# pyannote/pyannote-video

Measured on AMD Instinct MI355X. Metric: frames/sec end-to-end detect->embed->cluster, 1080p@25fps, higher is better.
Workload: dtype f32 (detector scores, embedder) / f64 (tracker, clustering) / u8 frames; an f16 screening pass with a proven error bound decides which windows the detector's exact f32 chain is evaluated for -- results identical to dense f32 scoring (`dense_scoring`)

## Files before the change

include/pvface.h:

```cpp
#ifndef PVFACE_H
#define PVFACE_H
#include <stdint.h>
#include <stddef.h>

#ifdef __cplusplus
extern "C" {
#endif

typedef uint64_t pvf_handle;
typedef struct { int32_t left, top, right, bottom; } pvf_rect_i32;

const char* pvf_last_error(void);
int32_t pvf_version(void);
int32_t pvf_device_count(int32_t* n);
int32_t pvf_ctx_create(int32_t device, pvf_handle* ctx);
int32_t pvf_ctx_create_prio(int32_t device, int32_t priority_class, pvf_handle* ctx);
int32_t pvf_ctx_destroy(pvf_handle ctx);
int32_t pvf_sync(pvf_handle ctx);

int32_t pvf_load_detector(pvf_handle ctx, const char* path);
int32_t pvf_load_shape_predictor(pvf_handle ctx, const char* path);
int32_t pvf_load_embedder(pvf_handle ctx, const char* path);
int32_t pvf_model_tensor(const char* path, int32_t kind, const char* name, void* out, int64_t cap_bytes, int64_t* nbytes);
int32_t pvf_set_tracker_tables(pvf_handle ctx, const double* mask64, const double* mask_scale, const double* tw64,
// ... 241 lines not shown
                        int32_t decimals, char* out, int64_t cap, int64_t* written);

int32_t pvf_round_rows(const float* x, int64_t n, int32_t decimals, double* out);

int32_t pvf_parse_rows(const char* text, int64_t len, double* out, int64_t cap, int64_t* n_rows, int32_t* n_cols);

int32_t pvf_prof_enable(pvf_handle ctx, int32_t on);
int32_t pvf_prof_reset(pvf_handle ctx);
int32_t pvf_prof_get(pvf_handle ctx, const char* family, double* total_ms, int64_t* launches);

int32_t pvf_debug_pyramid_level(pvf_handle ctx, pvf_handle frame, int32_t upsample, int32_t level,
                                uint8_t* out, int32_t* h, int32_t* w);
int32_t pvf_debug_pyramid_batch(pvf_handle ctx, const pvf_handle* frames, int32_t n, int32_t upsample);
int32_t pvf_debug_level_features(pvf_handle ctx, pvf_handle frame, int32_t upsample, int32_t level,
                                 float* out, int32_t* fh, int32_t* fw);
int32_t pvf_debug_level_plan(pvf_handle ctx, pvf_handle frame, int32_t upsample, int32_t level, int32_t* out8);
int32_t pvf_debug_fhog(pvf_handle ctx, const uint8_t* img, int32_t h, int32_t w, int32_t cell, int32_t pad_r,
                       int32_t pad_c, float* out, int32_t* fh, int32_t* fw);
int32_t pvf_debug_detect_raw(pvf_handle ctx, pvf_handle frame, int32_t upsample, double adjust, float* scores,
                             int32_t* meta , int32_t cap, int32_t* n);
int32_t pvf_debug_detect_raw_many(pvf_handle ctx, const pvf_handle* frames, int32_t n_frames, int32_t batch, int32_t upsample,
                                  double adjust, int32_t* counts, int32_t* rows, int64_t cap, int64_t* total);
int32_t pvf_debug_extract_chip(pvf_handle ctx, pvf_handle frame, const double rect[4], double cs, double sn,
                               int32_t rows, int32_t cols, uint8_t* out);
int32_t pvf_debug_tracker_state(pvf_handle ctx, pvf_handle trk, double* F, double* A, double* B);
int32_t pvf_debug_tracker_scale_state(pvf_handle ctx, pvf_handle trk, double* As, double* Bs);
int32_t pvf_debug_embed_stage(pvf_handle ctx, const uint8_t* chips, int32_t n, int32_t split, int32_t stage, float* out, int32_t dims[3],
                              int32_t* flags);
int32_t pvf_debug_conv(pvf_handle ctx, const int32_t geom[18], const float* in, const float* w, const float* bias, const float* gamma,
                       const float* beta, const float* skip, int32_t split, int32_t force_generic, float* out, int32_t* flags);
// ... 15 lines not shown
```

pyannote-video_amd/csrc/api.hip:

```cpp
#include "pvf_internal.h"
#include <algorithm>
#include <cmath>
#include <cstdlib>
#include <string>
#include <thread>

#define API_BEGIN try {
#define API_END                                                        \
    return 0;                                                          \
    }                                                                  \
    catch (const std::exception& e) { pvf_set_error(e.what()); return -1; } \
    catch (...) { pvf_set_error("unknown error"); return -2; }

#define ENTER(c, h)                                                \
    Ctx* c = pvf_ctx(h);                                           \
    std::lock_guard<std::recursive_mutex> _api_lock(c->api_mu);    \
    HIP_CHECK(hipSetDevice(c->device))
#define ENTER_DET(c, h)                                            \
    Ctx* c = pvf_ctx(h);                                           \
    std::lock_guard<std::recursive_mutex> _det_lock(c->det_mu);    \
    HIP_CHECK(hipSetDevice(c->device))
#define ENTER_BOTH(c, h)                                           \
    Ctx* c = pvf_ctx(h);                                           \
    std::lock_guard<std::recursive_mutex> _det_lock(c->det_mu);    \
// ... 185 lines not shown
    std::vector<Frame> fr;
    for (int i = 0; i < n; ++i) fr.push_back(c->frame(frames[i]));
    det_pyramid_batch(c, fr, upsample);
    API_END
}

extern "C" int32_t pvf_debug_level_features(pvf_handle h, pvf_handle frame, int32_t upsample, int32_t level, float* out, int32_t* fh, int32_t* fw)
{
    API_BEGIN
    ENTER_DET(c, h);
    std::vector<float> buf;
    int a = 0, b = 0;
    det_level_features(c, c->frame(frame), upsample, level, out ? &buf : nullptr, &a, &b);
    *fh = a; *fw = b;
    if (out) memcpy(out, buf.data(), buf.size() * sizeof(float));
    API_END
}

extern "C" int32_t pvf_debug_level_plan(pvf_handle h, pvf_handle frame, int32_t upsample, int32_t level, int32_t* out8)
{
    API_BEGIN
    ENTER_DET(c, h);
    PVF_REQUIRE(out8 != nullptr, "pvf_debug_level_plan: out8 is NULL");
    det_level_plan(c, c->frame(frame), upsample, level, out8);
    API_END
}

extern "C" int32_t pvf_debug_fhog(pvf_handle h, const uint8_t* img, int32_t ih, int32_t iw, int32_t cell, int32_t pad_r, int32_t pad_c,
                                  float* out, int32_t* fh, int32_t* fw)
{
// ... 1020 lines not shown
```

pyannote-video_amd/csrc/detect.hip:

```cpp
#include "detect_ml.h"
#include <algorithm>
#include <thread>
#include <cmath>
#include <cstdlib>

#define RESIZE_MAXS 22
struct RowTab { int32_t top, bottom; double tb, tb1, pad; };
struct ColTab { int32_t left, pad; double lr, lr1, pad2; };

template <int RS, int NSTRIP>
__global__ void __launch_bounds__(256) resize_rows_k(const uint8_t* const* __restrict__ in_ptrs, const uint8_t* __restrict__ in_base,
                                                     size_t in_stride, int in_rb, int ih, int iw, uint8_t* __restrict__ out,
                                                     size_t out_stride, int out_rb, int oh, int ow,
                                                     const RowTab* __restrict__ rows, const ColTab* __restrict__ cols)
{
    constexpr int MAXS = (RS == 16) ? RESIZE_MAXS : (RS * 5) / 4 + 3;
    __shared__ uint32_t s_rows[4][MAXS][64];
    __shared__ uint32_t s_out[4][64];
    const int lane = threadIdx.x & 63;
    const int wave = __builtin_amdgcn_readfirstlane(threadIdx.x >> 6);
    const int c0 = blockIdx.x * 256 + wave * 64;
    const int b = blockIdx.z;
    if (c0 >= ow) return;
    const int c = min(c0 + lane, ow - 1);
// ... 1007 lines not shown
                    memcpy(out->data() + ((size_t)y * d.fw + x) * PVF_FHOG_STRIDE + 4 * j, dev.data() + feat_at(y, j, x, d.fwp), 4 * sizeof(float));
    }
    HIP_CHECK(hipStreamSynchronize(c->det_stream));
}

void det_level_plan(Ctx* c, const Frame& f, int upsample, int level, int32_t out[8])
{
    PVF_REQUIRE(c->det.loaded, "detector not loaded");
    MlPlan* p = ml_plan(c, f.h, f.w, upsample, 1);
    PVF_REQUIRE(level >= 0 && level < (int)p->lv.size(), "pyramid level out of range");
    const LvDesc& d = p->lv[level];
    const int32_t v[8] = {d.h, d.w, d.hog_nr, d.hog_nc, d.chunk_rows, d.chunks, d.roll_rows, d.roll_nseg};
    memcpy(out, v, sizeof v);
}

static bool raw_less(const RawDet& x, const RawDet& y)
{
    if (x.score != y.score) return x.score > y.score;
    if (x.filter != y.filter) return x.filter < y.filter;
    if (x.level != y.level) return x.level < y.level;
    if (x.r != y.r) return x.r < y.r;
    return x.c < y.c;
}

static void decode_candidates(const DetectorModel& m, int upsample, const CandRec* q, int n, std::vector<RawDet>& v);

static void screen_verdict(Ctx* c, const int* ctl)
{
    if (!c->det_screen || c->det_screen_suspended) return;
    c->screen_listed += std::min(ctl[SCR_FLAGGED], c->screen_list_cap);
    if (ctl[SCR_FLAGGED] > c->screen_list_cap || ctl[SCR_VIOLATION] != 0) {
        HIP_CHECK(hipStreamSynchronize(c->det_stream));
        throw ScreenRetry();
    }
}

struct CandLayout { ScratchLayout lay; ScratchSlot<int> counts; ScratchSlot<CandRec> cands; };
static CandLayout cand_layout(int frames, int per_frame)
{
    CandLayout l;
    l.counts = l.lay.take<int>(frames + SCR_CTL_INTS, 64);
    l.cands = l.lay.take<CandRec>((size_t)frames * per_frame, 64);
    l.lay.pad(64);
    return l;
}

void det_run_batch(Ctx* c, const std::vector<Frame>& frames, int upsample, double adjust, std::vector<std::vector<RawDet>>& raw_sorted)
{
    const DetectorModel& m = c->det;
    PVF_REQUIRE(m.loaded, "detector not loaded");
    PVF_REQUIRE(!frames.empty(), "no frames");
    const int B = (int)frames.size();
    const int cap = c->det_cand_cap;
    const CandLayout cl = cand_layout(B, cap);
    c->s_cand.ensure(cl.lay.bytes());
    int* d_counts = cl.counts.in(c->s_cand); CandRec* d_cands = cl.cands.in(c->s_cand);
    HIP_CHECK(hipMemsetAsync(d_counts, 0, (size_t)(B + SCR_CTL_INTS) * sizeof(int), c->det_stream));
    ScoreParams sp;
    for (int f = 0; f < 8; ++f) sp.thresh[f] = f < m.n_filters ? (float)((double)m.thresh[f] + adjust) : 3.0e38f;
// ... 142 lines not shown
```

pyannote-video_amd/csrc/detect_ml.h:

```cpp
#pragma once
#include "pvf_internal.h"
#include "fhog_dev.h"

#define ML_MAX 32
struct LvDesc {
    int h, w, rb;
    int cells_nr, cells_nc, visible_nr, visible_nc;
    int fh, fw, hog_nr, hog_nc;
    int fwp;
    int feat_bx, score_bx;
    int valid_score;
    int roll_nseg, roll_rows;
    int strips, chunks, chunk_rows, fused_tasks;
    long long img_off, img_stride;
    long long feat_off, feat_stride;
};
struct MlStarts { int nl; int b0[ML_MAX + 1]; };

#define FEAT_PAD_COLS 52
__host__ __device__ __forceinline__ size_t feat_at(int row, int j, int col, int fwp) { return (((size_t)row * 8 + j) * fwp + col) * 4; }

struct ScoreParams { float thresh[8]; int n_filters; int level; int cap; };
struct CandRec { float score; int32_t filter, level, r, c; };

// ... 4 lines not shown
static_assert((SCR_GROUP_COLS - 1) + SCR_TAIL_CELLS - (SCR_FILTER_COLS - 1) <= FEAT_PAD_COLS,
              "FEAT_PAD_COLS: the screening pass's tail read leaves a feature row's zero columns");
struct ScreenItem { int32_t lv, b, c_base, r_base, out_rows, ng; };
enum { SCR_CURSOR = 0, SCR_FLAGGED = 1, SCR_VIOLATION = 2, SCR_CTL_INTS = 4 };

struct ScreenPlan {
    ScreenItem* d_items = nullptr;
    int n_items = 0;
    bool usable = false;
    ~ScreenPlan() { if (d_items) (void)hipFree(d_items); }
    ScreenPlan() = default;
    ScreenPlan(const ScreenPlan&) = delete;
    ScreenPlan& operator=(const ScreenPlan&) = delete;
};
void screen_plan_build(ScreenPlan& sp, const std::vector<LvDesc>& lv, int B);
void screen_launch(Ctx* c, const ScreenPlan& sp, const LvDesc* d_lv, int B, const float* feat, const ScoreParams& thr, int* d_counts,
                   CandRec* d_cands, int* ctl);
void screen_prepare_model(DetectorModel& d, const float* w);
```

pyannote-video_amd/csrc/pvf_internal.h:

```cpp
#pragma once
#include <hip/hip_runtime.h>
#include <cstdint>
#include <cstdio>
#include <cstring>
#include <deque>
#include <map>
#include <atomic>
#include <memory>
#include <mutex>
#include <stdexcept>
#include <string>
#include <unordered_map>
#include <vector>
#include "../../include/pvface.h"
#include "scratch_layout.h"
#include "chip_plan.h"
#include "group_blocks.h"

#define PVF_FHOG_STRIDE 32

struct CandOverflow : PvfError { int needed; explicit CandOverflow(int n) : PvfError("detector: candidate buffer overflow"), needed(n) {} };
struct ScreenRetry : PvfError { ScreenRetry() : PvfError("detector: screening pass gave up") {} };

#define HIP_CHECK(expr)                                                                              \
// ... 300 lines not shown
void det_run_many(Ctx* c, const std::vector<Frame>& frames, int batch, int upsample, double adjust,
                  std::vector<std::vector<RawDet>>& raw_sorted, bool nms = false);
void ml_plans_free(Ctx* c);
void ingest_free_all(Ctx* c);
struct ResizeTab { std::vector<int32_t> idx; std::vector<int16_t> coef; };
ResizeTab linear_table(int in, int out);
void render_free_all(Ctx* c);
void tube_free_all(Ctx* c);
void board_free_all(Ctx* c);
void board_thumbs_device(Ctx* c, const pvf_handle* frames, int n, int tw, int th, uint8_t* d_out);
int board_thumbs_per_round(size_t picture_bytes);
void det_nms(const DetectorModel& m, const std::vector<RawDet>& sorted, std::vector<RawDet>& out);
void det_pyramid_level(Ctx* c, const Frame& f, int upsample, int level, std::vector<uint8_t>* out, int* h, int* w);
void det_level_features(Ctx* c, const Frame& f, int upsample, int level, std::vector<float>* out, int* fh, int* fw);
void det_level_plan(Ctx* c, const Frame& f, int upsample, int level, int32_t out[8]);
void det_pyramid_batch(Ctx* c, const std::vector<Frame>& frames, int upsample);
void fhog_debug(Ctx* c, const uint8_t* himg, int h, int w, int cell, int pad_r, int pad_c, std::vector<float>& out, int* fh, int* fw);
void fhog_device(Ctx* c, const uint8_t* d_img, int n, int h, int w, int cell, int pad_r, int pad_c, float* d_feat,
                 DevBuf& hist, DevBuf& norm, size_t img_stride_in = 0);
void fhog1_compact(Ctx* c, const uint8_t* d_chips, int n, uint8_t* d_rec);
void fhog_scale_chips(Ctx* c, const uint8_t* d_chips, int n, float* d_feat);
void fhog_dims(int ih, int iw, int cell, int pad_r, int pad_c, int* fh, int* fw);
ChipJob chip_plan(const Frame& f, const ChipDetails& d);
void chip_extract_batch(Ctx* c, const std::vector<ChipJob>& jobs, uint8_t* d_out );
void transform_batch(Ctx* c, const std::vector<ChipJob>& jobs, uint8_t* d_out);
void transform_launch(Ctx* c, const DevXfJob* d_jobs, int n, int rows, int cols, uint8_t* d_out);
void jitter_check_count(const char* who, int J);
void jitter_plan_rows(int J, uint64_t seed, double* out );
int jitter_faces_per_round(int J);
uint8_t* jitter_scratch(Ctx* c, int faces, int J);
// ... 64 lines not shown
```

pyannote-video_amd/csrc/screen.hip:

```cpp
#include "detect_ml.h"
#include <algorithm>
#include <cmath>
#include <cstring>

typedef _Float16 f16x8 __attribute__((ext_vector_type(8)));
typedef _Float16 f16x2 __attribute__((ext_vector_type(2)));

struct ScreenParams { float flag_at[8]; float lim_lo, lim_hi; int n_items, list_cap; };

#define SCR_B_BYTES (10 * 12 * 64 * 16)
#define SCR_M_STRIDE (12 * 64 * 16)

__device__ __forceinline__ uint32_t pk_f16(float a, float b)
{
    return __builtin_bit_cast(uint32_t, __builtin_amdgcn_cvt_pkrtz(a, b));
}

template <int NG>
__device__ __forceinline__ void screen_walk(const ScreenItem t, const LvDesc* __restrict__ lv, const float* __restrict__ feat_base,
                                            const uint8_t* s_b, const float th_lane, int* __restrict__ ctl, uint2* __restrict__ list,
                                            const int list_cap, u32x4& mx)
{
    constexpr int RSRC_FLAGS = 0x00020000;
    constexpr int FR = 10, FC = 10;
    static_assert(FC == SCR_FILTER_COLS, "detect_ml.h: SCR_FILTER_COLS is this kernel's filter width");
    const int lane = threadIdx.x & 63, i = lane & 15, kq = lane >> 4;
    const int fw = lv[t.lv].fw;
    const long long feat_off = lv[t.lv].feat_off, feat_stride = lv[t.lv].feat_stride;
    const int fwp = lv[t.lv].fwp;
    const float* fb = feat_base + feat_off + (size_t)t.b * feat_stride + feat_at(t.r_base, 0, t.c_base, fwp);
    const int row_bytes = (8 * fwp - t.c_base) * 16;
    const int fh_in = t.out_rows + FR - 1;
    const int c1 = fw - (FC - FC / 2 - 1);
    const int voff = i * 48 + kq * 2 * fwp * 16;
    const int voff2 = voff + fwp * 16;
    const int voff_t = i < 3 ? voff : 0x40000000, voff2_t = i < 3 ? voff2 : 0x40000000;
    f32x4 acc[10][NG];
#pragma unroll
    for (int q = 0; q < 10; ++q)
#pragma unroll
        for (int g = 0; g < NG; ++g) acc[q][g] = (f32x4){0.f, 0.f, 0.f, 0.f};
    const uint8_t* b_lo = s_b + lane * 16;
    const uint8_t* b_hi = s_b + lane * 16 + 5 * SCR_M_STRIDE;
    auto load_cls = [&](int row, int cls, u32x4 (&raw)[NG + 1][2]) {
        const __amdgpu_buffer_rsrc_t rs = __builtin_amdgcn_make_buffer_rsrc((void*)(fb + (size_t)row * 8 * fwp * 4), 0,
                                                                            row < fh_in ? row_bytes : 0, RSRC_FLAGS);
#pragma unroll
        for (int g = 0; g <= NG; ++g) {
            raw[g][0] = __builtin_amdgcn_raw_buffer_load_b128(rs, (g < NG ? voff : voff_t) + cls * 16 + g * 768, 0, 0);
            raw[g][1] = __builtin_amdgcn_raw_buffer_load_b128(rs, (g < NG ? voff2 : voff2_t) + cls * 16 + g * 768, 0, 0);
        }
    };
    auto cvt_frag = [&](const u32x4 (&r)[2]) -> u32x4 {
        u32x4 o;
        o.x = pk_f16(__uint_as_float(r[0].x), __uint_as_float(r[0].y)); o.y = pk_f16(__uint_as_float(r[0].z), __uint_as_float(r[0].w));
        o.z = pk_f16(__uint_as_float(r[1].x), __uint_as_float(r[1].y)); o.w = pk_f16(__uint_as_float(r[1].z), __uint_as_float(r[1].w));
#pragma unroll
        for (int k = 0; k < 4; ++k) mx[k] = __builtin_bit_cast(uint32_t, __builtin_elementwise_max(__builtin_bit_cast(f16x2, mx[k]), __builtin_bit_cast(f16x2, o[k])));
        return o;
    };
    auto shift_bases = [&](u32x4 (&a)[NG + 1]) {
#pragma unroll
        for (int g = 0; g <= NG; ++g) {
#pragma unroll
            for (int e = 0; e < 4; ++e) {
                int fill = 0;
                if (g < NG) fill = __builtin_amdgcn_update_dpp(0, (int)a[g + 1][e], 0x11F , 0xf, 0xf, true);
                a[g][e] = (uint32_t)__builtin_amdgcn_update_dpp(fill, (int)a[g][e], 0x101 , 0xf, 0xf, false);
            }
        }
    };
    auto emit = [&](const f32x4 (&a)[NG], int r_out) {
        float vm = a[0][0];
#pragma unroll
        for (int g = 0; g < NG; ++g)
#pragma unroll
            for (int e = 0; e < 4; ++e) vm = fmaxf(vm, a[g][e]);
        const bool hit = vm >= th_lane;
        if (r_out >= 0 && __builtin_amdgcn_ballot_w64(hit) != 0) {
            const int jc = lane & 15;
            const int sft = jc / 5, f = jc % 5;
            const int r = t.r_base + r_out + FR / 2;
#pragma unroll
            for (int g = 0; g < NG; ++g)
#pragma unroll
                for (int e = 0; e < 4; ++e) {
                    const int cc = t.c_base + 48 * g + 3 * (4 * kq + e) + sft + FC / 2;
                    if (a[g][e] >= th_lane && cc < c1) {
                        const int idx = atomicAdd(&ctl[SCR_FLAGGED], 1);
                        if (idx < list_cap) list[idx] = make_uint2((uint32_t)t.b, ((uint32_t)t.lv << 27) | ((uint32_t)f << 24) | ((uint32_t)r << 12) | (uint32_t)cc);
                    }
                }
        }
    };

    u32x4 A[3][NG + 1];
    {
        u32x4 raw[NG + 1][2];
#pragma unroll
        for (int cls = 0; cls < 3; ++cls) {
            load_cls(0, cls, raw);
#pragma unroll
            for (int g = 0; g <= NG; ++g) A[cls][g] = cvt_frag(raw[g]);
        }
    }
    auto b_frag = [&](int q, int j) -> u32x4 {
        return *reinterpret_cast<const u32x4*>((q < 5 ? b_lo + q * SCR_M_STRIDE : b_hi + (q - 5) * SCR_M_STRIDE) + j * 1024);
    };
    u32x4 bn[10];
#pragma unroll
    for (int q = 0; q < 10; ++q) bn[q] = b_frag(q, 0);
    for (int s = 0; s < fh_in; ++s) {
        u32x4 An[3][NG + 1];
        u32x4 raw[NG + 1][2];
        f32x4 done[NG];
#pragma unroll
        for (int j = 0; j < 12; ++j) {
            const int cls = j % 3;
            if (j > 0 && cls == 0) {
#pragma unroll
                for (int k = 0; k < 3; ++k) shift_bases(A[k]);
            }
            if (j % 4 == 0) load_cls(s + 1, j / 4, raw);
            u32x4 bc[10];
#pragma unroll
            for (int q = 0; q < 10; ++q) bc[q] = bn[q];
#pragma unroll
            for (int q = 0; q < 10; ++q) bn[q] = b_frag(q, (j + 1) % 12);
#pragma unroll
            for (int q = 9; q >= 0; --q) {
#pragma unroll
                for (int g = 0; g < NG; ++g) {
                    const f32x4 v = __builtin_amdgcn_mfma_f32_16x16x32_f16(__builtin_bit_cast(f16x8, A[cls][g]), __builtin_bit_cast(f16x8, bc[q]), acc[q][g], 0, 0, 0);
                    if (j < 11) acc[q][g] = v;
                    else if (q == 9) done[g] = v;
                    else acc[q + 1][g] = v;
                }
            }
            if (j % 4 == 3) {
#pragma unroll
                for (int g = 0; g <= NG; ++g) An[j / 4][g] = cvt_frag(raw[g]);
            }
            __builtin_amdgcn_sched_barrier(0);
        }
#pragma unroll
        for (int g = 0; g < NG; ++g) acc[0][g] = (f32x4){0.f, 0.f, 0.f, 0.f};
        emit(done, s - (FR - 1));
#pragma unroll
        for (int cls = 0; cls < 3; ++cls)
#pragma unroll
            for (int g = 0; g <= NG; ++g) A[cls][g] = An[cls][g];
    }
}

__global__ void __launch_bounds__(256) __attribute__((amdgpu_waves_per_eu(1, 1)))
score_screen_k(const ScreenItem* __restrict__ items, const LvDesc* __restrict__ lv, const float* __restrict__ feat_base,
               const u32x4* __restrict__ Bh, ScreenParams sp, int* __restrict__ ctl, uint2* __restrict__ list)
{
    extern __shared__ __attribute__((aligned(16))) uint8_t s_b[];
    for (int k = threadIdx.x; k < SCR_B_BYTES / 16; k += 256) reinterpret_cast<u32x4*>(s_b)[k] = Bh[k];
    __syncthreads();
    const int lane = threadIdx.x & 63;
    const int jc = lane & 15, f = jc % 5;
    float th_lane = sp.flag_at[0];
    th_lane = f == 1 ? sp.flag_at[1] : th_lane;
    th_lane = f == 2 ? sp.flag_at[2] : th_lane;
    th_lane = f == 3 ? sp.flag_at[3] : th_lane;
    th_lane = f == 4 ? sp.flag_at[4] : th_lane;
    th_lane = jc < 15 ? th_lane : 3.0e38f;
    u32x4 mx = {0u, 0u, 0u, 0u};
    for (;;) {
        int it = 0;
        if (lane == 0) it = atomicAdd(&ctl[SCR_CURSOR], 1);
        it = __builtin_amdgcn_readfirstlane(it);
        if (it >= sp.n_items) break;
        ScreenItem t;
        t.lv = __builtin_amdgcn_readfirstlane(items[it].lv); t.b = __builtin_amdgcn_readfirstlane(items[it].b);
        t.c_base = __builtin_amdgcn_readfirstlane(items[it].c_base); t.r_base = __builtin_amdgcn_readfirstlane(items[it].r_base);
        t.out_rows = __builtin_amdgcn_readfirstlane(items[it].out_rows); t.ng = __builtin_amdgcn_readfirstlane(items[it].ng);
        switch (t.ng) {
        case 1: screen_walk<1>(t, lv, feat_base, s_b, th_lane, ctl, list, sp.list_cap, mx); break;
        case 2: screen_walk<2>(t, lv, feat_base, s_b, th_lane, ctl, list, sp.list_cap, mx); break;
        case 3: screen_walk<3>(t, lv, feat_base, s_b, th_lane, ctl, list, sp.list_cap, mx); break;
        default: screen_walk<4>(t, lv, feat_base, s_b, th_lane, ctl, list, sp.list_cap, mx); break;
        }
    }
    auto lo16 = [](uint32_t v) { return (float)__builtin_bit_cast(f16x2, v)[0]; };
    auto hi16 = [](uint32_t v) { return (float)__builtin_bit_cast(f16x2, v)[1]; };
    const float m_lo = fmaxf(fmaxf(lo16(mx.x), hi16(mx.x)), lo16(mx.y));
    const float m_hi = fmaxf(fmaxf(hi16(mx.y), fmaxf(lo16(mx.z), hi16(mx.z))), fmaxf(lo16(mx.w), hi16(mx.w)));
    const float lim_hi = (lane >> 4) == 3 ? sp.lim_hi : sp.lim_lo;
    if (m_lo > sp.lim_lo || m_hi > lim_hi) atomicOr(&ctl[SCR_VIOLATION], 1);
}

__global__ void __launch_bounds__(256) score_list_k(const uint2* __restrict__ list, const int* __restrict__ ctl, int list_cap,
                                                    const LvDesc* __restrict__ lv, const float* __restrict__ feat_base,
                                                    const float* __restrict__ W, ScoreParams sp, int* __restrict__ counts, CandRec* __restrict__ cands)
{
    constexpr int FR = 10, FC = 10;
    const int n = min(ctl[SCR_FLAGGED], list_cap);
    for (int e = blockIdx.x * 256 + threadIdx.x; e < n; e += gridDim.x * 256) {
        const uint2 q = list[e];
        const int b = (int)q.x;
        const int l = (int)(q.y >> 27), f = (int)((q.y >> 24) & 7), r = (int)((q.y >> 12) & 4095), cc = (int)(q.y & 4095);
        const int fwp = lv[l].fwp;
        const float* fp = feat_base + lv[l].feat_off + (size_t)b * lv[l].feat_stride + feat_at(r - FR / 2, 0, cc - FC / 2, fwp);
        const float* wp = W + (size_t)f * FR * FC * PVF_FHOG_STRIDE;
        float acc = 0.0f;
        for (int m = 0; m < FR; ++m)
            for (int nn = 0; nn < FC; ++nn) {
                const f32x4* fv = reinterpret_cast<const f32x4*>(fp + feat_at(m, 0, nn, fwp));
                const f32x4* wv = reinterpret_cast<const f32x4*>(wp + ((size_t)m * FC + nn) * PVF_FHOG_STRIDE);
#pragma unroll
                for (int k = 0; k < 8; ++k) {
                    const f32x4 a = fv[(size_t)k * fwp], w = wv[k];
                    acc = fmaf(a[0], w[0], acc); acc = fmaf(a[1], w[1], acc); acc = fmaf(a[2], w[2], acc);
                    if (k < 7) acc = fmaf(a[3], w[3], acc);
                }
            }
        const float th = sp.thresh[f];
        if (acc >= th) {
            const int idx = atomicAdd(&counts[b], 1);
            if (idx < sp.cap) {
                CandRec rec;
                rec.score = acc - th; rec.filter = f; rec.level = l; rec.r = r; rec.c = cc;
                cands[(size_t)b * sp.cap + idx] = rec;
            }
        }
    }
}

__global__ void screen_probe_k(const u32x4* __restrict__ a, const u32x4* __restrict__ b, int steps, float* __restrict__ d, int* __restrict__ moved)
{
    const int lane = threadIdx.x;
// ... 221 lines not shown
        worst = std::max(worst, worst_rel());
    }
    {
        for (size_t i = 0; i < nh; ++i) { ha[i] = 0x3c00u ; hb[i] = 0x0010u ; }
        run();
        c->screen_pipe_flushes_subnormals = !(hd[0] > 0.0f);
        if (!c->screen_pipe_flushes_subnormals) worst = std::max(worst, worst_rel());
    }
    (void)hipFree(dev);
    c->screen_pipe_err = worst;
    PVF_REQUIRE(worst <= 3200.0 * std::ldexp(1.0, -22), "screening: v_mfma_f32_16x16x32_f16 does not accumulate as the error bound of the screening pass assumes on this device");
    PVF_REQUIRE(dpp_ok, "screening: v_mov_b32_dpp row_shl:1 / row_shr:15 do not move data as the screening kernel expects on this device");
}

void screen_launch(Ctx* c, const ScreenPlan& plan, const LvDesc* d_lv, int B, const float* feat, const ScoreParams& thr, int* d_counts,
                   CandRec* d_cands, int* ctl)
{
    const DetectorModel& m = c->det;
    if (plan.n_items == 0) return;
    if (!c->screen_attr_set) {
        screen_probe(c);
        HIP_CHECK(hipFuncSetAttribute(reinterpret_cast<const void*>(score_screen_k), hipFuncAttributeMaxDynamicSharedMemorySize, SCR_B_BYTES));
        c->screen_attr_set = true;
    }
    ScreenParams sp;
    for (int f = 0; f < 8; ++f) {
        if (f < m.n_filters) {
            const float at = (float)(((double)thr.thresh[f] - m.screen_bound[f]) * m.screen_scale);
            sp.flag_at[f] = std::nextafterf(at, -INFINITY);
        }
        else sp.flag_at[f] = 3.0e38f;
    }
    sp.lim_lo = SCR_LIM_LO; sp.lim_hi = SCR_LIM_HI;
    if (const char* e = getenv("PVF_SCREEN_LIMIT_SCALE")) {
        sp.lim_lo *= (float)atof(e); sp.lim_hi *= (float)atof(e);
    }
    sp.n_items = plan.n_items;
    sp.list_cap = c->screen_list_cap;
    c->s_screen.ensure((size_t)sp.list_cap * sizeof(uint2) + 64);
    uint2* list = c->s_screen.as<uint2>();
    const int grid = std::min(c->n_cu, (plan.n_items + 3) / 4);
    hipLaunchKernelGGL(score_screen_k, dim3(grid), dim3(256), SCR_B_BYTES, c->det_stream, plan.d_items, d_lv, feat,
                       reinterpret_cast<const u32x4*>(m.d_bscreen), sp, ctl, list);
    hipLaunchKernelGGL(score_list_k, dim3(256), dim3(256), 0, c->det_stream, list, ctl, sp.list_cap, d_lv, feat, m.d_w, thr, d_counts, d_cands);
}
```

pyannote-video_amd/pyannote_video_amd/_lib.py:

```python
import ctypes as C
import os
import numpy as np

_HERE = os.path.dirname(os.path.abspath(__file__))
LIB_PATH = os.environ.get("PVF_LIBRARY") or os.path.join(_HERE, "libpvface.so")

_lib = None


class PvfError(RuntimeError):
    pass


class OrbCapError(PvfError):

    def __init__(self, message, needed):
        PvfError.__init__(self, message)
        self.needed = int(needed)


class Rect(C.Structure):
    _fields_ = [("left", C.c_int32), ("top", C.c_int32), ("right", C.c_int32), ("bottom", C.c_int32)]


# ... 113 lines not shown
    "pvf_cast_plan": (C.c_int32, [C.c_int64, C.c_int32, P]),
    "pvf_frame_prints": (C.c_int32, [H, P, C.c_int32, P, C.c_int32]),
    "pvf_print_runs": (C.c_int32, [H, P, P, C.c_int32, P, P, C.c_int32, C.c_int32, C.c_int32, C.c_int32, P, C.c_int64, P]),
    "pvf_frame_blend": (C.c_int32, [H, P, C.c_int32, C.c_int32, C.c_int32, P, C.c_int32, P, P]),
    "pvf_blend_measure": (C.c_int32, [H, P, C.c_int32, C.c_int32, C.c_int32, P]),
    "pvf_format_rows": (C.c_int32, [P, P, P, C.c_int64, C.c_int32, C.c_int32, P, C.c_int64, P]),
    "pvf_round_rows": (C.c_int32, [P, C.c_int64, C.c_int32, P]),
    "pvf_parse_rows": (C.c_int32, [C.c_char_p, C.c_int64, P, C.c_int64, P, P]),
    "pvf_prof_enable": (C.c_int32, [H, C.c_int32]),
    "pvf_prof_reset": (C.c_int32, [H]),
    "pvf_prof_get": (C.c_int32, [H, C.c_char_p, P, P]),
    "pvf_debug_pyramid_level": (C.c_int32, [H, H, C.c_int32, C.c_int32, P, P, P]),
    "pvf_debug_pyramid_batch": (C.c_int32, [H, P, C.c_int32, C.c_int32]),
    "pvf_debug_level_features": (C.c_int32, [H, H, C.c_int32, C.c_int32, P, P, P]),
    "pvf_debug_level_plan": (C.c_int32, [H, H, C.c_int32, C.c_int32, P]),
    "pvf_debug_fhog": (C.c_int32, [H, P, C.c_int32, C.c_int32, C.c_int32, C.c_int32, C.c_int32, P, P, P]),
    "pvf_debug_detect_raw": (C.c_int32, [H, H, C.c_int32, C.c_double, P, P, C.c_int32, P]),
    "pvf_debug_detect_raw_many": (C.c_int32, [H, P, C.c_int32, C.c_int32, C.c_int32, C.c_double, P, P, C.c_int64, P]),
    "pvf_debug_extract_chip": (C.c_int32, [H, H, P, C.c_double, C.c_double, C.c_int32, C.c_int32, P]),
    "pvf_debug_tracker_state": (C.c_int32, [H, H, P, P, P]),
    "pvf_debug_tracker_scale_state": (C.c_int32, [H, H, P, P]),
    "pvf_debug_embed_stage": (C.c_int32, [H, P, C.c_int32, C.c_int32, C.c_int32, P, P, P]),
    "pvf_debug_conv": (C.c_int32, [H, P, P, P, P, P, P, P, C.c_int32, C.c_int32, P, P]),
    "pvf_debug_embed_head": (C.c_int32, [H, P, C.c_int32, C.c_int32, P]),
    "pvf_shot_dfd": (C.c_int32, [H, P, C.c_int32, C.c_int32, C.c_int32, P, P, P, P]),
    "pvf_orb_extract": (C.c_int32, [H, P, C.c_int32, C.c_int32, C.c_int32, C.c_int32, P, P, P]),
    "pvf_orb_match_counts": (C.c_int32, [H, P, P, C.c_int32, C.c_int32, P, C.c_int64, P]),
}
EXPORTS = sorted(_SIGS)

# ... 146 lines not shown
```

pyannote-video_amd/pyannote_video_amd/runtime.py:

```python
import contextlib
import ctypes as C
import threading
import itertools
import operator
import numpy as np
from . import _lib
from ._lib import check, ptr, handles
from . import models as _models
from .y4m import YuvFrame, chroma_shape


class DeviceFrame(object):
    __slots__ = ("ctx", "handle", "height", "width", "keep", "transient", "__weakref__")

    def __init__(self, ctx, handle, height, width, keep=None, transient=False):
        self.ctx, self.handle, self.height, self.width, self.keep = ctx, handle, height, width, keep
        self.transient = transient

    @property
    def shape(self):
        return (self.height, self.width, 3)

    def release(self):
        if self.handle is not None and self.ctx._h is not None:
# ... 501 lines not shown
    def pyramid_level(self, frame, upsample, level):
        f = self.stage(frame)
        oh, ow = C.c_int32(0), C.c_int32(0)
        check(self._l.pvf_debug_pyramid_level(self._h, f.handle, upsample, level, None, C.byref(oh), C.byref(ow)))
        out = np.zeros((oh.value, ow.value, 3), np.uint8)
        check(self._l.pvf_debug_pyramid_level(self._h, f.handle, upsample, level, ptr(out), C.byref(oh), C.byref(ow)))
        return out

    def level_features(self, frame, upsample, level):
        f = self.stage(frame)
        fh, fw = C.c_int32(0), C.c_int32(0)
        check(self._l.pvf_debug_level_features(self._h, f.handle, upsample, level, None, C.byref(fh), C.byref(fw)))
        out = np.zeros((fh.value, fw.value, 32), np.float32)
        if out.size:
            check(self._l.pvf_debug_level_features(self._h, f.handle, upsample, level, ptr(out), C.byref(fh), C.byref(fw)))
        return out

    def level_plan(self, frame, upsample, level):
        f = self.stage(frame)
        out = np.zeros(8, np.int32)
        check(self._l.pvf_debug_level_plan(self._h, f.handle, int(upsample), int(level), ptr(out)))
        return dict(zip(("h", "w", "hog_nr", "hog_nc", "chunk_rows", "chunks", "roll_rows", "roll_nseg"), (int(v) for v in out)))

    def fhog(self, img, cell, pad_r, pad_c):
        img = np.ascontiguousarray(img, np.uint8)
        fh, fw = C.c_int32(0), C.c_int32(0)
        check(self._l.pvf_debug_fhog(self._h, ptr(img), img.shape[0], img.shape[1], cell, pad_r, pad_c, None, C.byref(fh), C.byref(fw)))
        out = np.zeros((fh.value, fw.value, 32), np.float32)
        check(self._l.pvf_debug_fhog(self._h, ptr(img), img.shape[0], img.shape[1], cell, pad_r, pad_c, ptr(out), C.byref(fh), C.byref(fw)))
        return out
# ... 725 lines not shown
```

Before: 4906.

## Restructure screen MFMA walk loads and stage exact rescoring weights in LDS

The f16 screening walk now issues all three class loads for the next row up front and splits the B-fragment prefetch into two halves, so each half's MFMAs overlap the next half's LDS reads and register pressure drops. The f16 max-tracking that feeds the error-bound check drops the unused w component and moves into the walk. The exact f32 rescoring kernel becomes 64-thread blocks that copy the filter weights into shared memory once, with a rotating feature-cell prefetch. A debug entry point that dumps the screening sums is also added. This trades more register and LDS staging complexity for better latency hiding. Changing the max computation also touches the error-bound check and could affect correctness if the bound was relying on the dropped lanes.

```diff
diff --git a/include/pvface.h b/include/pvface.h
--- a/include/pvface.h
+++ b/include/pvface.h
@@ -279,6 +279,7 @@
 int32_t pvf_debug_pyramid_batch(pvf_handle ctx, const pvf_handle* frames, int32_t n, int32_t upsample);
 int32_t pvf_debug_level_features(pvf_handle ctx, pvf_handle frame, int32_t upsample, int32_t level,
                                  float* out, int32_t* fh, int32_t* fw);
+int32_t pvf_debug_screen_sums(pvf_handle ctx, pvf_handle frame, int32_t upsample, int32_t level, float* out);
 int32_t pvf_debug_level_plan(pvf_handle ctx, pvf_handle frame, int32_t upsample, int32_t level, int32_t* out8);
 int32_t pvf_debug_fhog(pvf_handle ctx, const uint8_t* img, int32_t h, int32_t w, int32_t cell, int32_t pad_r,
                        int32_t pad_c, float* out, int32_t* fh, int32_t* fw);
diff --git a/pyannote-video_amd/csrc/api.hip b/pyannote-video_amd/csrc/api.hip
--- a/pyannote-video_amd/csrc/api.hip
+++ b/pyannote-video_amd/csrc/api.hip
@@ -223,6 +223,15 @@
     det_level_features(c, c->frame(frame), upsample, level, out ? &buf : nullptr, &a, &b);
     *fh = a; *fw = b;
     if (out) memcpy(out, buf.data(), buf.size() * sizeof(float));
+    API_END
+}
+
+extern "C" int32_t pvf_debug_screen_sums(pvf_handle h, pvf_handle frame, int32_t upsample, int32_t level, float* out)
+{
+    API_BEGIN
+    ENTER_DET(c, h);
+    PVF_REQUIRE(upsample >= 0 && upsample <= 2, "pvf_debug_screen_sums: upsample must be 0..2");
+    det_screen_sums(c, c->frame(frame), upsample, level, out);
     API_END
 }
 
diff --git a/pyannote-video_amd/csrc/detect.hip b/pyannote-video_amd/csrc/detect.hip
--- a/pyannote-video_amd/csrc/detect.hip
+++ b/pyannote-video_amd/csrc/detect.hip
@@ -1045,6 +1045,23 @@
     memcpy(out, v, sizeof v);
 }
 
+struct CandLayout;
+static CandLayout cand_layout(int frames, int per_frame);
+static void screen_sums_run(Ctx* c, MlPlan* p, int level, float* out);
+
+void det_screen_sums(Ctx* c, const Frame& f, int upsample, int level, float* out)
+{
+    PVF_REQUIRE(c->det.loaded, "detector not loaded");
+    PVF_REQUIRE(out != nullptr, "pvf_debug_screen_sums: out is NULL");
+    std::vector<Frame> fr{f};
+    MlPlan* p = ml_features(c, fr, upsample);
+    PVF_REQUIRE(level >= 0 && level < (int)p->lv.size(), "pyramid level out of range");
+    PVF_REQUIRE(p->lv[level].valid_score && p->walk_blocks > 0, "pvf_debug_screen_sums: the level has no window");
+    if (!p->screen_built) { screen_plan_build(p->screen, p->lv, 1); p->screen_built = true; }
+    PVF_REQUIRE(p->screen.usable, "pvf_debug_screen_sums: the screening pass does not take this plan");
+    screen_sums_run(c, p, level, out);
+}
+
 static bool raw_less(const RawDet& x, const RawDet& y)
 {
     if (x.score != y.score) return x.score > y.score;
@@ -1074,6 +1091,31 @@
     l.cands = l.lay.take<CandRec>((size_t)frames * per_frame, 64);
     l.lay.pad(64);
     return l;
+}
+
+static void screen_sums_run(Ctx* c, MlPlan* p, int level, float* out)
+{
+    const DetectorModel& m = c->det;
+    const LvDesc& d = p->lv[level];
+    const size_t n = (size_t)(d.fh - 9) * (d.fw - 9) * 5;
+    const int cap = c->det_cand_cap;
+    const CandLayout cl = cand_layout(1, cap);
+    c->s_cand.ensure(cl.lay.bytes());
+    int* d_counts = cl.counts.in(c->s_cand); CandRec* d_cands = cl.cands.in(c->s_cand);
+    HIP_CHECK(hipMemsetAsync(d_counts, 0, (size_t)(1 + SCR_CTL_INTS) * sizeof(int), c->det_stream));
+    ScoreParams sp;
+    for (int f = 0; f < 8; ++f) sp.thresh[f] = f < m.n_filters ? m.thresh[f] : 3.0e38f;
+    sp.n_filters = m.n_filters; sp.cap = cap;
+    float* d_out = nullptr;
+    HIP_CHECK(hipMalloc((void**)&d_out, n * sizeof(float)));
+    HIP_CHECK(hipMemsetAsync(d_out, 0xff, n * sizeof(float), c->det_stream));
+    const ScreenDebug dbg{d_out, level, 0};
+    screen_launch(c, p->screen, p->d_lv, 1, c->s_feat.as<float>(), sp, d_counts, d_cands, d_counts + 1, &dbg);
+    const hipError_t e1 = hipMemcpyAsync(out, d_out, n * sizeof(float), hipMemcpyDeviceToHost, c->det_stream);
+    const hipError_t e2 = hipStreamSynchronize(c->det_stream);
+    (void)hipFree(d_out);
+    HIP_CHECK(e1);
+    HIP_CHECK(e2);
 }
 
 void det_run_batch(Ctx* c, const std::vector<Frame>& frames, int upsample, double adjust, std::vector<std::vector<RawDet>>& raw_sorted)
diff --git a/pyannote-video_amd/csrc/detect_ml.h b/pyannote-video_amd/csrc/detect_ml.h
--- a/pyannote-video_amd/csrc/detect_ml.h
+++ b/pyannote-video_amd/csrc/detect_ml.h
@@ -42,6 +42,7 @@
     ScreenPlan& operator=(const ScreenPlan&) = delete;
 };
 void screen_plan_build(ScreenPlan& sp, const std::vector<LvDesc>& lv, int B);
+struct ScreenDebug { float* out; int level, frame; };
 void screen_launch(Ctx* c, const ScreenPlan& sp, const LvDesc* d_lv, int B, const float* feat, const ScoreParams& thr, int* d_counts,
-                   CandRec* d_cands, int* ctl);
+                   CandRec* d_cands, int* ctl, const ScreenDebug* dbg = nullptr);
 void screen_prepare_model(DetectorModel& d, const float* w);
diff --git a/pyannote-video_amd/csrc/pvf_internal.h b/pyannote-video_amd/csrc/pvf_internal.h
--- a/pyannote-video_amd/csrc/pvf_internal.h
+++ b/pyannote-video_amd/csrc/pvf_internal.h
@@ -338,6 +338,7 @@
 void det_pyramid_level(Ctx* c, const Frame& f, int upsample, int level, std::vector<uint8_t>* out, int* h, int* w);
 void det_level_features(Ctx* c, const Frame& f, int upsample, int level, std::vector<float>* out, int* fh, int* fw);
 void det_level_plan(Ctx* c, const Frame& f, int upsample, int level, int32_t out[8]);
+void det_screen_sums(Ctx* c, const Frame& f, int upsample, int level, float* out);
 void det_pyramid_batch(Ctx* c, const std::vector<Frame>& frames, int upsample);
 void fhog_debug(Ctx* c, const uint8_t* himg, int h, int w, int cell, int pad_r, int pad_c, std::vector<float>& out, int* fh, int* fw);
 void fhog_device(Ctx* c, const uint8_t* d_img, int n, int h, int w, int cell, int pad_r, int pad_c, float* d_feat,
diff --git a/pyannote-video_amd/csrc/screen.hip b/pyannote-video_amd/csrc/screen.hip
--- a/pyannote-video_amd/csrc/screen.hip
+++ b/pyannote-video_amd/csrc/screen.hip
@@ -6,7 +6,7 @@
 typedef _Float16 f16x8 __attribute__((ext_vector_type(8)));
 typedef _Float16 f16x2 __attribute__((ext_vector_type(2)));
 
-struct ScreenParams { float flag_at[8]; float lim_lo, lim_hi; int n_items, list_cap; };
+struct ScreenParams { float flag_at[8]; float lim_lo, lim_hi; int n_items, list_cap; float* dbg; float dbg_mul; int dbg_lv, dbg_b; };
 
 #define SCR_B_BYTES (10 * 12 * 64 * 16)
 #define SCR_M_STRIDE (12 * 64 * 16)
@@ -16,15 +16,30 @@
     return __builtin_bit_cast(uint32_t, __builtin_amdgcn_cvt_pkrtz(a, b));
 }
 
+__device__ __forceinline__ int lane_here()
+{
+    int l = (int)__builtin_amdgcn_mbcnt_hi(~0u, __builtin_amdgcn_mbcnt_lo(~0u, 0u));
+    asm volatile("" : "+v"(l));
+    return l;
+}
+
 template <int NG>
 __device__ __forceinline__ void screen_walk(const ScreenItem t, const LvDesc* __restrict__ lv, const float* __restrict__ feat_base,
-                                            const uint8_t* s_b, const float th_lane, int* __restrict__ ctl, uint2* __restrict__ list,
-                                            const int list_cap, u32x4& mx)
+                                            const uint8_t* s_b, const ScreenParams& sp, int* __restrict__ ctl, uint2* __restrict__ list)
 {
     constexpr int RSRC_FLAGS = 0x00020000;
     constexpr int FR = 10, FC = 10;
     static_assert(FC == SCR_FILTER_COLS, "detect_ml.h: SCR_FILTER_COLS is this kernel's filter width");
-    const int lane = threadIdx.x & 63, i = lane & 15, kq = lane >> 4;
+    const int lane = lane_here();
+    const int i = lane & 15, kq = lane >> 4;
+    const int list_cap = sp.list_cap;
+    float th_lane = sp.flag_at[0];
+    th_lane = i % 5 == 1 ? sp.flag_at[1] : th_lane;
+    th_lane = i % 5 == 2 ? sp.flag_at[2] : th_lane;
+    th_lane = i % 5 == 3 ? sp.flag_at[3] : th_lane;
+    th_lane = i % 5 == 4 ? sp.flag_at[4] : th_lane;
+    th_lane = i < 15 ? th_lane : 3.0e38f;
+    u32x4 mx = {0u, 0u, 0u, 0u};
     const int fw = lv[t.lv].fw;
     const long long feat_off = lv[t.lv].feat_off, feat_stride = lv[t.lv].feat_stride;
     const int fwp = lv[t.lv].fwp;
@@ -33,8 +48,8 @@
     const int fh_in = t.out_rows + FR - 1;
     const int c1 = fw - (FC - FC / 2 - 1);
     const int voff = i * 48 + kq * 2 * fwp * 16;
-    const int voff2 = voff + fwp * 16;
-    const int voff_t = i < 3 ? voff : 0x40000000, voff2_t = i < 3 ? voff2 : 0x40000000;
+    const int soff2 = fwp * 16;
+    const int voff_t = i < 3 ? voff : 0x40000000;
     f32x4 acc[10][NG];
 #pragma unroll
     for (int q = 0; q < 10; ++q)
@@ -42,21 +57,23 @@
         for (int g = 0; g < NG; ++g) acc[q][g] = (f32x4){0.f, 0.f, 0.f, 0.f};
     const uint8_t* b_lo = s_b + lane * 16;
     const uint8_t* b_hi = s_b + lane * 16 + 5 * SCR_M_STRIDE;
-    auto load_cls = [&](int row, int cls, u32x4 (&raw)[NG + 1][2]) {
+    auto load_row = [&](int row, u32x4 (&raw)[3][NG + 1][2]) {
         const __amdgpu_buffer_rsrc_t rs = __builtin_amdgcn_make_buffer_rsrc((void*)(fb + (size_t)row * 8 * fwp * 4), 0,
                                                                             row < fh_in ? row_bytes : 0, RSRC_FLAGS);
 #pragma unroll
         for (int g = 0; g <= NG; ++g) {
-            raw[g][0] = __builtin_amdgcn_raw_buffer_load_b128(rs, (g < NG ? voff : voff_t) + cls * 16 + g * 768, 0, 0);
-            raw[g][1] = __builtin_amdgcn_raw_buffer_load_b128(rs, (g < NG ? voff2 : voff2_t) + cls * 16 + g * 768, 0, 0);
+#pragma unroll
+            for (int cls = 0; cls < 3; ++cls) raw[cls][g][0] = __builtin_amdgcn_raw_buffer_load_b128(rs, (g < NG ? voff : voff_t) + cls * 16 + g * 768, 0, 0);
+#pragma unroll
+            for (int cls = 0; cls < 3; ++cls) raw[cls][g][1] = __builtin_amdgcn_raw_buffer_load_b128(rs, (g < NG ? voff : voff_t) + cls * 16 + g * 768, soff2, 0);
         }
     };
     auto cvt_frag = [&](const u32x4 (&r)[2]) -> u32x4 {
         u32x4 o;
         o.x = pk_f16(__uint_as_float(r[0].x), __uint_as_float(r[0].y)); o.y = pk_f16(__uint_as_float(r[0].z), __uint_as_float(r[0].w));
         o.z = pk_f16(__uint_as_float(r[1].x), __uint_as_float(r[1].y)); o.w = pk_f16(__uint_as_float(r[1].z), __uint_as_float(r[1].w));
-#pragma unroll
-        for (int k = 0; k < 4; ++k) mx[k] = __builtin_bit_cast(uint32_t, __builtin_elementwise_max(__builtin_bit_cast(f16x2, mx[k]), __builtin_bit_cast(f16x2, o[k])));
+        auto pk_max = [](uint32_t a, uint32_t b) { return __builtin_bit_cast(uint32_t, __builtin_elementwise_max(__builtin_bit_cast(f16x2, a), __builtin_bit_cast(f16x2, b))); };
+        mx.x = pk_max(mx.x, o.x); mx.y = pk_max(mx.y, o.y); mx.z = pk_max(mx.z, pk_max(o.z, o.w));
         return o;
     };
     auto shift_bases = [&](u32x4 (&a)[NG + 1]) {
@@ -77,8 +94,21 @@
 #pragma unroll
             for (int e = 0; e < 4; ++e) vm = fmaxf(vm, a[g][e]);
         const bool hit = vm >= th_lane;
+        if (sp.dbg != nullptr && r_out >= 0 && t.lv == sp.dbg_lv && t.b == sp.dbg_b) {
+            const int lane_d = lane_here();
+            const int jc = lane_d & 15, kq = lane_d >> 4;
+#pragma unroll
+            for (int g = 0; g < NG; ++g)
+#pragma unroll
+                for (int e = 0; e < 4; ++e) {
+                    const int col = t.c_base + 48 * g + 3 * (4 * kq + e) + jc / 5;
+                    if (jc < 15 && col < fw - (FC - 1))
+                        sp.dbg[((size_t)(t.r_base + r_out) * (fw - (FC - 1)) + col) * 5 + jc % 5] = a[g][e] * sp.dbg_mul;
+                }
+        }
         if (r_out >= 0 && __builtin_amdgcn_ballot_w64(hit) != 0) {
-            const int jc = lane & 15;
+            const int lane_e = lane_here();
+            const int jc = lane_e & 15, kq = lane_e >> 4;
             const int sft = jc / 5, f = jc % 5;
             const int r = t.r_base + r_out + FR / 2;
 #pragma unroll
@@ -95,62 +125,67 @@
     };
 
     u32x4 A[3][NG + 1];
-    {
-        u32x4 raw[NG + 1][2];
-#pragma unroll
-        for (int cls = 0; cls < 3; ++cls) {
-            load_cls(0, cls, raw);
-#pragma unroll
-            for (int g = 0; g <= NG; ++g) A[cls][g] = cvt_frag(raw[g]);
-        }
-    }
+    u32x4 raw[3][NG + 1][2];
+    load_row(0, raw);
+#pragma unroll
+    for (int cls = 0; cls < 3; ++cls)
+#pragma unroll
+        for (int g = 0; g <= NG; ++g) A[cls][g] = cvt_frag(raw[cls][g]);
     auto b_frag = [&](int q, int j) -> u32x4 {
         return *reinterpret_cast<const u32x4*>((q < 5 ? b_lo + q * SCR_M_STRIDE : b_hi + (q - 5) * SCR_M_STRIDE) + j * 1024);
     };
-    u32x4 bn[10];
-#pragma unroll
-    for (int q = 0; q < 10; ++q) bn[q] = b_frag(q, 0);
+    u32x4 bhi[5], blo[5];
+#pragma unroll
+    for (int q = 0; q < 5; ++q) { blo[q] = b_frag(q, 0); bhi[q] = b_frag(q + 5, 0); }
     for (int s = 0; s < fh_in; ++s) {
-        u32x4 An[3][NG + 1];
-        u32x4 raw[NG + 1][2];
         f32x4 done[NG];
+        load_row(s + 1, raw);
 #pragma unroll
         for (int j = 0; j < 12; ++j) {
             const int cls = j % 3;
-            if (j > 0 && cls == 0) {
-#pragma unroll
-                for (int k = 0; k < 3; ++k) shift_bases(A[k]);
-            }
-            if (j % 4 == 0) load_cls(s + 1, j / 4, raw);
-            u32x4 bc[10];
-#pragma unroll
-            for (int q = 0; q < 10; ++q) bc[q] = bn[q];
-#pragma unroll
-            for (int q = 0; q < 10; ++q) bn[q] = b_frag(q, (j + 1) % 12);
-#pragma unroll
-            for (int q = 9; q >= 0; --q) {
+            if (j >= 1 && j <= 9) shift_bases(A[(j - 1) % 3]);
+            u32x4 nhi[5], nlo[5];
+#pragma unroll
+            for (int q = 0; q < 5; ++q) nhi[q] = b_frag(q + 5, (j + 1) % 12);
+#pragma unroll
+            for (int q = 9; q >= 5; --q) {
 #pragma unroll
                 for (int g = 0; g < NG; ++g) {
-                    const f32x4 v = __builtin_amdgcn_mfma_f32_16x16x32_f16(__builtin_bit_cast(f16x8, A[cls][g]), __builtin_bit_cast(f16x8, bc[q]), acc[q][g], 0, 0, 0);
+                    const f32x4 v = __builtin_amdgcn_mfma_f32_16x16x32_f16(__builtin_bit_cast(f16x8, A[cls][g]), __builtin_bit_cast(f16x8, bhi[q - 5]), acc[q][g], 0, 0, 0);
                     if (j < 11) acc[q][g] = v;
                     else if (q == 9) done[g] = v;
                     else acc[q + 1][g] = v;
                 }
             }
-            if (j % 4 == 3) {
-#pragma unroll
-                for (int g = 0; g <= NG; ++g) An[j / 4][g] = cvt_frag(raw[g]);
+#pragma unroll
+            for (int q = 0; q < 5; ++q) nlo[q] = b_frag(q, (j + 1) % 12);
+#pragma unroll
+            for (int q = 4; q >= 0; --q) {
+#pragma unroll
+                for (int g = 0; g < NG; ++g) {
+                    const f32x4 v = __builtin_amdgcn_mfma_f32_16x16x32_f16(__builtin_bit_cast(f16x8, A[cls][g]), __builtin_bit_cast(f16x8, blo[q]), acc[q][g], 0, 0, 0);
+                    if (j < 11) acc[q][g] = v;
+                    else acc[q + 1][g] = v;
+                }
+            }
+#pragma unroll
+            for (int q = 0; q < 5; ++q) { bhi[q] = nhi[q]; blo[q] = nlo[q]; }
+            if (j >= 9) {
+#pragma unroll
+                for (int g = 0; g <= NG; ++g) A[j - 9][g] = cvt_frag(raw[j - 9][g]);
             }
             __builtin_amdgcn_sched_barrier(0);
         }
 #pragma unroll
         for (int g = 0; g < NG; ++g) acc[0][g] = (f32x4){0.f, 0.f, 0.f, 0.f};
         emit(done, s - (FR - 1));
-#pragma unroll
-        for (int cls = 0; cls < 3; ++cls)
-#pragma unroll
-            for (int g = 0; g <= NG; ++g) A[cls][g] = An[cls][g];
-    }
+    }
+    auto lo16 = [](uint32_t v) { return (float)__builtin_bit_cast(f16x2, v)[0]; };
+    auto hi16 = [](uint32_t v) { return (float)__builtin_bit_cast(f16x2, v)[1]; };
+    const float m_lo = fmaxf(fmaxf(lo16(mx.x), hi16(mx.x)), lo16(mx.y));
+    const float m_hi = fmaxf(hi16(mx.y), fmaxf(lo16(mx.z), hi16(mx.z)));
+    const float lim_hi = (lane_here() >> 4) == 3 ? sp.lim_hi : sp.lim_lo;
+    if (m_lo > sp.lim_lo || m_hi > lim_hi) atomicOr(&ctl[SCR_VIOLATION], 1);
 }
 
 __global__ void __launch_bounds__(256) __attribute__((amdgpu_waves_per_eu(1, 1)))
@@ -160,18 +195,9 @@
     extern __shared__ __attribute__((aligned(16))) uint8_t s_b[];
     for (int k = threadIdx.x; k < SCR_B_BYTES / 16; k += 256) reinterpret_cast<u32x4*>(s_b)[k] = Bh[k];
     __syncthreads();
-    const int lane = threadIdx.x & 63;
-    const int jc = lane & 15, f = jc % 5;
-    float th_lane = sp.flag_at[0];
-    th_lane = f == 1 ? sp.flag_at[1] : th_lane;
-    th_lane = f == 2 ? sp.flag_at[2] : th_lane;
-    th_lane = f == 3 ? sp.flag_at[3] : th_lane;
-    th_lane = f == 4 ? sp.flag_at[4] : th_lane;
-    th_lane = jc < 15 ? th_lane : 3.0e38f;
-    u32x4 mx = {0u, 0u, 0u, 0u};
     for (;;) {
         int it = 0;
-        if (lane == 0) it = atomicAdd(&ctl[SCR_CURSOR], 1);
+        if (lane_here() == 0) it = atomicAdd(&ctl[SCR_CURSOR], 1);
         it = __builtin_amdgcn_readfirstlane(it);
         if (it >= sp.n_items) break;
         ScreenItem t;
@@ -179,45 +205,62 @@
         t.c_base = __builtin_amdgcn_readfirstlane(items[it].c_base); t.r_base = __builtin_amdgcn_readfirstlane(items[it].r_base);
         t.out_rows = __builtin_amdgcn_readfirstlane(items[it].out_rows); t.ng = __builtin_amdgcn_readfirstlane(items[it].ng);
         switch (t.ng) {
-        case 1: screen_walk<1>(t, lv, feat_base, s_b, th_lane, ctl, list, sp.list_cap, mx); break;
-        case 2: screen_walk<2>(t, lv, feat_base, s_b, th_lane, ctl, list, sp.list_cap, mx); break;
-        case 3: screen_walk<3>(t, lv, feat_base, s_b, th_lane, ctl, list, sp.list_cap, mx); break;
-        default: screen_walk<4>(t, lv, feat_base, s_b, th_lane, ctl, list, sp.list_cap, mx); break;
-        }
-    }
-    auto lo16 = [](uint32_t v) { return (float)__builtin_bit_cast(f16x2, v)[0]; };
-    auto hi16 = [](uint32_t v) { return (float)__builtin_bit_cast(f16x2, v)[1]; };
-    const float m_lo = fmaxf(fmaxf(lo16(mx.x), hi16(mx.x)), lo16(mx.y));
-    const float m_hi = fmaxf(fmaxf(hi16(mx.y), fmaxf(lo16(mx.z), hi16(mx.z))), fmaxf(lo16(mx.w), hi16(mx.w)));
-    const float lim_hi = (lane >> 4) == 3 ? sp.lim_hi : sp.lim_lo;
-    if (m_lo > sp.lim_lo || m_hi > lim_hi) atomicOr(&ctl[SCR_VIOLATION], 1);
-}
-
-__global__ void __launch_bounds__(256) score_list_k(const uint2* __restrict__ list, const int* __restrict__ ctl, int list_cap,
-                                                    const LvDesc* __restrict__ lv, const float* __restrict__ feat_base,
-                                                    const float* __restrict__ W, ScoreParams sp, int* __restrict__ counts, CandRec* __restrict__ cands)
-{
-    constexpr int FR = 10, FC = 10;
+        case 1: screen_walk<1>(t, lv, feat_base, s_b, sp, ctl, list); break;
+        case 2: screen_walk<2>(t, lv, feat_base, s_b, sp, ctl, list); break;
+        case 3: screen_walk<3>(t, lv, feat_base, s_b, sp, ctl, list); break;
+        default: screen_walk<4>(t, lv, feat_base, s_b, sp, ctl, list); break;
+        }
+    }
+}
+
+#define LIST_AHEAD 5
+#define LIST_BLOCKS 1024
+__global__ void __launch_bounds__(64) score_list_k(const uint2* __restrict__ list, const int* __restrict__ ctl, int list_cap,
+                                                   const LvDesc* __restrict__ lv, const float* __restrict__ feat_base,
+                                                   const float* __restrict__ W, ScoreParams sp, int* __restrict__ counts, CandRec* __restrict__ cands)
+{
+    constexpr int FR = 10, FC = 10, D = LIST_AHEAD;
+    static_assert(FC % D == 0, "the cells of a filter row take turns in the D feature buffers");
+    __shared__ f32x4 s_w[5 * FR * FC * 8];
     const int n = min(ctl[SCR_FLAGGED], list_cap);
-    for (int e = blockIdx.x * 256 + threadIdx.x; e < n; e += gridDim.x * 256) {
+    if ((int)blockIdx.x * 64 >= n) return;
+    for (int k = threadIdx.x; k < 5 * FR * FC * 8; k += 64) s_w[k] = reinterpret_cast<const f32x4*>(W)[k];
+    __syncthreads();
+    for (int e = blockIdx.x * 64 + threadIdx.x; e < n; e += gridDim.x * 64) {
         const uint2 q = list[e];
         const int b = (int)q.x;
         const int l = (int)(q.y >> 27), f = (int)((q.y >> 24) & 7), r = (int)((q.y >> 12) & 4095), cc = (int)(q.y & 4095);
         const int fwp = lv[l].fwp;
         const float* fp = feat_base + lv[l].feat_off + (size_t)b * lv[l].feat_stride + feat_at(r - FR / 2, 0, cc - FC / 2, fwp);
-        const float* wp = W + (size_t)f * FR * FC * PVF_FHOG_STRIDE;
+        const f32x4* wl = s_w + f * (FR * FC * 8);
+        auto cell = [&](int m, int nn, f32x4 (&dst)[8]) {
+            const f32x4* fv = reinterpret_cast<const f32x4*>(fp + feat_at(m, 0, nn, fwp));
+#pragma unroll
+            for (int k = 0; k < 8; ++k) dst[k] = fv[(size_t)k * fwp];
+        };
+        f32x4 fa[D][8], wc[8], wn[8];
+#pragma unroll
+        for (int d = 0; d < D; ++d) cell(0, d, fa[d]);
+#pragma unroll
+        for (int k = 0; k < 8; ++k) wc[k] = wl[k];
         float acc = 0.0f;
-        for (int m = 0; m < FR; ++m)
+        for (int m = 0; m < FR; ++m) {
+#pragma unroll
             for (int nn = 0; nn < FC; ++nn) {
-                const f32x4* fv = reinterpret_cast<const f32x4*>(fp + feat_at(m, 0, nn, fwp));
-                const f32x4* wv = reinterpret_cast<const f32x4*>(wp + ((size_t)m * FC + nn) * PVF_FHOG_STRIDE);
+                const int next = min(m * FC + nn + 1, FR * FC - 1);
+#pragma unroll
+                for (int k = 0; k < 8; ++k) wn[k] = wl[next * 8 + k];
 #pragma unroll
                 for (int k = 0; k < 8; ++k) {
-                    const f32x4 a = fv[(size_t)k * fwp], w = wv[k];
+                    const f32x4 a = fa[nn % D][k], w = wc[k];
                     acc = fmaf(a[0], w[0], acc); acc = fmaf(a[1], w[1], acc); acc = fmaf(a[2], w[2], acc);
                     if (k < 7) acc = fmaf(a[3], w[3], acc);
                 }
-            }
+                cell(nn + D < FC ? m : min(m + 1, FR - 1), (nn + D) % FC, fa[nn % D]);
+#pragma unroll
+                for (int k = 0; k < 8; ++k) wc[k] = wn[k];
+            }
+        }
         const float th = sp.thresh[f];
         if (acc >= th) {
             const int idx = atomicAdd(&counts[b], 1);
@@ -469,7 +512,7 @@
 }
 
 void screen_launch(Ctx* c, const ScreenPlan& plan, const LvDesc* d_lv, int B, const float* feat, const ScoreParams& thr, int* d_counts,
-                   CandRec* d_cands, int* ctl)
+                   CandRec* d_cands, int* ctl, const ScreenDebug* dbg)
 {
     const DetectorModel& m = c->det;
     if (plan.n_items == 0) return;
@@ -492,10 +535,13 @@
     }
     sp.n_items = plan.n_items;
     sp.list_cap = c->screen_list_cap;
+    sp.dbg = dbg ? dbg->out : nullptr;
+    sp.dbg_mul = (float)(1.0 / m.screen_scale);
+    sp.dbg_lv = dbg ? dbg->level : -1; sp.dbg_b = dbg ? dbg->frame : -1;
     c->s_screen.ensure((size_t)sp.list_cap * sizeof(uint2) + 64);
     uint2* list = c->s_screen.as<uint2>();
     const int grid = std::min(c->n_cu, (plan.n_items + 3) / 4);
     hipLaunchKernelGGL(score_screen_k, dim3(grid), dim3(256), SCR_B_BYTES, c->det_stream, plan.d_items, d_lv, feat,
                        reinterpret_cast<const u32x4*>(m.d_bscreen), sp, ctl, list);
-    hipLaunchKernelGGL(score_list_k, dim3(256), dim3(256), 0, c->det_stream, list, ctl, sp.list_cap, d_lv, feat, m.d_w, thr, d_counts, d_cands);
-}
+    hipLaunchKernelGGL(score_list_k, dim3(LIST_BLOCKS), dim3(64), 0, c->det_stream, list, ctl, sp.list_cap, d_lv, feat, m.d_w, thr, d_counts, d_cands);
+}
diff --git a/pyannote-video_amd/pyannote_video_amd/_lib.py b/pyannote-video_amd/pyannote_video_amd/_lib.py
--- a/pyannote-video_amd/pyannote_video_amd/_lib.py
+++ b/pyannote-video_amd/pyannote_video_amd/_lib.py
@@ -151,6 +151,7 @@
     "pvf_debug_pyramid_batch": (C.c_int32, [H, P, C.c_int32, C.c_int32]),
     "pvf_debug_level_features": (C.c_int32, [H, H, C.c_int32, C.c_int32, P, P, P]),
     "pvf_debug_level_plan": (C.c_int32, [H, H, C.c_int32, C.c_int32, P]),
+    "pvf_debug_screen_sums": (C.c_int32, [H, H, C.c_int32, C.c_int32, P]),
     "pvf_debug_fhog": (C.c_int32, [H, P, C.c_int32, C.c_int32, C.c_int32, C.c_int32, C.c_int32, P, P, P]),
     "pvf_debug_detect_raw": (C.c_int32, [H, H, C.c_int32, C.c_double, P, P, C.c_int32, P]),
     "pvf_debug_detect_raw_many": (C.c_int32, [H, P, C.c_int32, C.c_int32, C.c_int32, C.c_double, P, P, C.c_int64, P]),
diff --git a/pyannote-video_amd/pyannote_video_amd/runtime.py b/pyannote-video_amd/pyannote_video_amd/runtime.py
--- a/pyannote-video_amd/pyannote_video_amd/runtime.py
+++ b/pyannote-video_amd/pyannote_video_amd/runtime.py
@@ -539,6 +539,16 @@
         out = np.zeros((fh.value, fw.value, 32), np.float32)
         if out.size:
             check(self._l.pvf_debug_level_features(self._h, f.handle, upsample, level, ptr(out), C.byref(fh), C.byref(fw)))
+        return out
+
+    def screen_sums(self, frame, upsample, level):
+        f = self.stage(frame)
+        fh, fw = C.c_int32(0), C.c_int32(0)
+        check(self._l.pvf_debug_level_features(self._h, f.handle, int(upsample), int(level), None, C.byref(fh), C.byref(fw)))
+        if fh.value < 10 or fw.value < 10:
+            raise ValueError("level %d has no window" % level)
+        out = np.zeros((fh.value - 9, fw.value - 9, 5), np.float32)
+        check(self._l.pvf_debug_screen_sums(self._h, f.handle, int(upsample), int(level), ptr(out)))
         return out
 
     def level_plan(self, frame, upsample, level):
```

After: 4860. Within noise of the previous version (-0.9%).
